# TuringLang/Bijectors.jl

Measured on NVIDIA H100. Metric: samples/sec: with_logabsdet_jacobian through 8-layer Planar flow, D=128, higher is better.
Workload: dtype f32

## Files before the change

bijectors.jl_b200/csrc/b2b_planar_const.cu:

```cuda
#include "b2b_planar_common.cuh"

namespace b2b {

template <int D>
struct PlanarHP {
  float v[2 * HP_MAX_L * D + 2 * HP_MAX_L];
};

template <int D>
struct ArgSrc {
  static constexpr bool kDerive = false;
  const PlanarHP<D>& H;
  int invmask;
  __device__ __forceinline__ bool inv(int l) const { return (invmask >> l) & 1; }
};

struct DevSrc {
  static constexpr bool kDerive = true;
  int invmask;
  __device__ __forceinline__ bool inv(int l) const { return (invmask >> l) & 1; }
};

template <int D, int DIR, bool MVN, class Src>
struct PlanarProg {
  using State = V1NoState;
  const Src src;
  const B2BChainParams& P;
  const int L;
  static constexpr bool DERIVE = Src::kDerive;
  static constexpr bool TAB = DERIVE && DIR != 0;
  __device__ __forceinline__ int npk() const { return 2 * L * D + 2 * L; }
  __device__ __forceinline__ int mvn_off() const { return (npk() + 3) & ~3; }
  __device__ __forceinline__ int tab_off() const { return mvn_off() + (MVN ? 2 * D + 4 : 0); }

  __device__ __forceinline__ void stage(float* params, int warp, int lane, int nw) const {
    if constexpr (DERIVE) {
      if (MVN && warp == nw - 1) stage_layer(P.layers[L], params + mvn_off(), D, D, lane);
      planar_derive_smem<D>(P, L, L, params, warp, lane, nw);
      if constexpr (TAB) {
        __syncthreads();
        for (int idx = warp * 32 + lane; idx < L * PT_N; idx += nw * 32) {
          const int l = idx / PT_N;
          if (DIR == 1 || src.inv(l)) planar_table_piece(params[2 * L * D + l], idx - l * PT_N, params + tab_off() + l * PT_FLOATS);
        }
      }
    } else {
      for (int i = warp * 32 + lane; i < npk(); i += nw * 32) params[i] = src.H.v[i];
    }
  }

  __device__ __forceinline__ void apply(float2 (&x)[1][D / 2], const ColCtx<D, 1>& ctx, const float* params,
                                        float (&lj)[1]) const {
    const float* cb = params + 2 * L * D;
    const float* tab = params + tab_off();
#pragma unroll 1
    for (int l = 0; l < L; ++l) {
      const float4* w4 = reinterpret_cast<const float4*>(params + l * D);
      const float4* u4 = reinterpret_cast<const float4*>(params + (L + l) * D);
      float2 acc[4];
#pragma unroll
      for (int i = 0; i < 4; ++i) acc[i] = make_float2(0.f, 0.f);
#pragma unroll
      for (int i = 0; i < D / 4; ++i) {
        const float4 w = w4[i];
        acc[(i & 1) * 2 + 0] = b2b_ffma2(make_float2(w.x, w.y), x[0][2 * i], acc[(i & 1) * 2 + 0]);
        acc[(i & 1) * 2 + 1] = b2b_ffma2(make_float2(w.z, w.w), x[0][2 * i + 1], acc[(i & 1) * 2 + 1]);
      }
      const float2 s = b2b_fadd2(b2b_fadd2(acc[0], acc[1]), b2b_fadd2(acc[2], acc[3]));
      const float wz = s.x + s.y;
      const float cc_ = cb[l], bb = cb[L + l];
      float t, s2;
      if (DIR == 0 || (DIR == 2 && !src.inv(l))) {
        tanh_sech2(wz + bb, t, s2);
        lj[0] += log1pf(cc_ * s2);
      } else {
        if constexpr (TAB) find_alpha_tab(wz, cc_, bb, tab + l * PT_FLOATS, t, s2);
        else find_alpha_ts(wz, cc_, bb, t, s2);
        lj[0] -= log1pf(cc_ * s2);
        t = -t;
      }
      const float2 t2 = make_float2(t, t);
#pragma unroll
      for (int i = 0; i < D / 4; ++i) {
        const float4 u = u4[i];
        x[0][2 * i] = b2b_ffma2(make_float2(u.x, u.y), t2, x[0][2 * i]);
        x[0][2 * i + 1] = b2b_ffma2(make_float2(u.z, u.w), t2, x[0][2 * i + 1]);
      }
    }
    if (MVN) mvnormal_apply<D, 1, 1>(x, ctx, params + mvn_off(), lj);
  }
};

template <int D, int NW, int DIR>
__global__ void __launch_bounds__(NW * 32, 1)
    planar_arg_kernel(const __grid_constant__ B2BChainParams P, const __grid_constant__ V1Extra E,
                      const __grid_constant__ CUtensorMap map_x, const __grid_constant__ CUtensorMap map_y,
                      const __grid_constant__ PlanarHP<D> H, const int L, const int invmask) {
  const PlanarProg<D, DIR, false, ArgSrc<D>> prog{{H, invmask}, P, L};
  v1_run<D, 1, 1, NW>(P, E, map_x, map_y, prog);
}

template <int D, int NW, int DIR, bool MVN>
__global__ void __launch_bounds__(NW * 32, 1)
    planar_dev_kernel(const __grid_constant__ B2BChainParams P, const __grid_constant__ V1Extra E,
                      const __grid_constant__ CUtensorMap map_x, const __grid_constant__ CUtensorMap map_y,
                      const int L, const int invmask) {
  const PlanarProg<D, DIR, MVN, DevSrc> prog{{invmask}, P, L};
  v1_run<D, 1, 1, NW>(P, E, map_x, map_y, prog);
}

template <int D, int NW, int DIR>
static int launch_arg(const B2BChainParams& q, const V1Geom& g, const CUtensorMap& mx, const CUtensorMap& my, int L,
                      const float* packed, int invmask, cudaStream_t stream) {
  static PlanarHP<D> H;
  static std::mutex mu;
  std::lock_guard<std::mutex> lock(mu);
  memcpy(H.v, packed, sizeof(float) * (size_t)(2 * L * D + 2 * L));
  auto kernel = planar_arg_kernel<D, NW, DIR>;
  cudaError_t e = cudaFuncSetAttribute(kernel, cudaFuncAttributeMaxDynamicSharedMemorySize, (int)g.smem);
  if (e != cudaSuccess) return (int)e;
  kernel<<<g.grid, NW * 32, g.smem, stream>>>(q, g.extra, mx, my, H, L, invmask);
  return (int)cudaGetLastError();
}

template <int D, int NW, int DIR, bool MVN = false>
static int launch_dev(const B2BChainParams& q, const V1Geom& g, const CUtensorMap& mx, const CUtensorMap& my, int L,
                      int invmask, cudaStream_t stream) {
  auto kernel = planar_dev_kernel<D, NW, DIR, MVN>;
  cudaError_t e = cudaFuncSetAttribute(kernel, cudaFuncAttributeMaxDynamicSharedMemorySize, (int)g.smem);
  if (e != cudaSuccess) return (int)e;
  kernel<<<g.grid, NW * 32, g.smem, stream>>>(q, g.extra, mx, my, L, invmask);
  return (int)cudaGetLastError();
}

template <int D, int NW>
static int dispatch(int L, const B2BChainParams& q, const V1Geom& g, const CUtensorMap& mx, const CUtensorMap& my,
                    const float* packed, int invmask, bool mvn, cudaStream_t stream) {
  const int all = (1 << L) - 1;
  const int dir = (invmask & all) == 0 ? 0 : ((invmask & all) == all ? 1 : 2);
  if (packed) {
    if (dir == 0) return launch_arg<D, NW, 0>(q, g, mx, my, L, packed, invmask, stream);
    if (dir == 1) return launch_arg<D, NW, 1>(q, g, mx, my, L, packed, invmask, stream);
    return launch_arg<D, NW, 2>(q, g, mx, my, L, packed, invmask, stream);
  }
  if (mvn) {
    if (dir == 1) return launch_dev<D, NW, 1, true>(q, g, mx, my, L, invmask, stream);
    return B2B_EUNSUPPORTED;
  }
  if (dir == 0) return launch_dev<D, NW, 0>(q, g, mx, my, L, invmask, stream);
  if (dir == 1) return launch_dev<D, NW, 1>(q, g, mx, my, L, invmask, stream);
  return launch_dev<D, NW, 2>(q, g, mx, my, L, invmask, stream);
}

static int launch_planar(const B2BChainParams& p, int L, const float* packed, int invmask, bool mvn,
                                  cudaStream_t stream) {
  B2BChainParams q = p;
  q.scratch_off = -1;
  if (!(q.D == 32 || q.D == 64 || q.D == 128) || L < 1 || L > HP_MAX_L) return B2B_EUNSUPPORTED;
  if (v1_check_io(q) != 0) return B2B_EUNSUPPORTED;
  V1Geom g;
  const size_t pf = (size_t)((2 * L * q.D + 2 * L + 3) & ~3) + (mvn ? 2 * q.D + 4 : 0) +
                    ((!packed && invmask != 0) ? (size_t)L * PT_FLOATS : 0);
  const int rc = v1_geometry(q.D, q.N, hp_warps(q.D), 32, pf, g);
  if (rc != 0) return rc;
  CUtensorMap mx, my;
  if (!make_maps(q, g.cols, &mx, &my, &g.extra.tma3d)) return B2B_EUNSUPPORTED;
  if (q.D == 128) return dispatch<128, 8>(L, q, g, mx, my, packed, invmask, mvn, stream);
  if (q.D == 64) return dispatch<64, 12>(L, q, g, mx, my, packed, invmask, mvn, stream);
  return dispatch<32, 16>(L, q, g, mx, my, packed, invmask, mvn, stream);
}

}

int b2b_planar_const_grid_size(const B2BChainParams& p) {
  using namespace b2b;
  if (!(p.D == 32 || p.D == 64 || p.D == 128)) return 0;
  V1Geom g;
  if (v1_geometry(p.D, p.N, hp_warps(p.D), 32, 0, g) != 0) return 0;
  return g.grid;
}

int b2b_launch_planar_hostparams(const B2BChainParams& p, int L, const float* packed, int invmask,
                                 cudaStream_t stream) {
  return b2b::launch_planar(p, L, packed, invmask, false, stream);
}

int b2b_planar_const_layers(const B2BChainParams& p) {
  using namespace b2b;
  if (!(p.D == 32 || p.D == 64 || p.D == 128) || p.L < 1) return 0;
  const bool mvn = p.layers[p.L - 1].kind == B2B_MVNORMAL_DIAG;
  const int n = p.L - (mvn ? 1 : 0);
  if (n < 1 || n > HP_MAX_L) return 0;
  for (int l = 0; l < n; ++l) {
    if (p.layers[l].kind != B2B_PLANAR) return 0;
    if (mvn && !p.layers[l].inverse) return 0;
  }
  if (v1_check_io(p) != 0) return 0;
  return n;
}

int b2b_launch_planar_chain_const(const B2BChainParams& p, cudaStream_t stream) {
  using namespace b2b;
  const int n = b2b_planar_const_layers(p);
  if (n == 0) return B2B_EUNSUPPORTED;
  int invmask = 0;
  for (int l = 0; l < n; ++l)
    if (p.layers[l].inverse) invmask |= 1 << l;
  return launch_planar(p, n, nullptr, invmask, p.L > n, stream);
}
```

bijectors.jl_b200/csrc/b2b_v1_pipeline.cuh:

```cuda
#pragma once
#include <cuda.h>
#include <cuda_runtime.h>

#include <cstdlib>
#include <mutex>

#include "b2b_device.cuh"

namespace b2b {

__device__ __forceinline__ uint32_t smem_u32(const void* p) {
  return static_cast<uint32_t>(__cvta_generic_to_shared(p));
}
__device__ __forceinline__ void mbar_init(uint32_t bar, uint32_t count) {
  asm volatile("mbarrier.init.shared::cta.b64 [%0], %1;" ::"r"(bar), "r"(count));
}
__device__ __forceinline__ void mbar_expect_tx(uint32_t bar, uint32_t bytes) {
  asm volatile("mbarrier.arrive.expect_tx.shared::cta.b64 _, [%0], %1;" ::"r"(bar), "r"(bytes) : "memory");
}
__device__ __forceinline__ void mbar_wait(uint32_t bar, uint32_t parity) {
  asm volatile(
      "{\n"
      ".reg .pred P1;\n"
      "B2B_WAIT:\n"
      "mbarrier.try_wait.parity.shared::cta.b64 P1, [%0], %1;\n"
      "@P1 bra B2B_DONE;\n"
      "bra B2B_WAIT;\n"
      "B2B_DONE:\n"
      "}\n" ::"r"(bar),
      "r"(parity)
      : "memory");
}
__device__ __forceinline__ void tma_load_2d(uint32_t dst, const CUtensorMap* map, int c0, int c1, uint32_t bar) {
  asm volatile(
      "cp.async.bulk.tensor.2d.shared::cluster.global.mbarrier::complete_tx::bytes [%0], [%1, {%2, %3}], [%4];" ::"r"(dst),
      "l"(reinterpret_cast<uint64_t>(map)), "r"(c0), "r"(c1), "r"(bar)
      : "memory");
}
__device__ __forceinline__ void tma_store_2d(const CUtensorMap* map, int c0, int c1, uint32_t src, uint64_t pol) {
  asm volatile("cp.async.bulk.tensor.2d.global.shared::cta.bulk_group.L2::cache_hint [%0, {%1, %2}], [%3], %4;" ::"l"(
                   reinterpret_cast<uint64_t>(map)),
               "r"(c0), "r"(c1), "r"(src), "l"(pol)
               : "memory");
}
__device__ __forceinline__ void tma_load_3d(uint32_t dst, const CUtensorMap* map, int c0, int c1, int c2, uint32_t bar) {
  asm volatile(
      "cp.async.bulk.tensor.3d.shared::cluster.global.mbarrier::complete_tx::bytes [%0], [%1, {%2, %3, %4}], [%5];" ::"r"(dst),
      "l"(reinterpret_cast<uint64_t>(map)), "r"(c0), "r"(c1), "r"(c2), "r"(bar)
      : "memory");
}
__device__ __forceinline__ void tma_store_3d(const CUtensorMap* map, int c0, int c1, int c2, uint32_t src, uint64_t pol) {
  asm volatile("cp.async.bulk.tensor.3d.global.shared::cta.bulk_group.L2::cache_hint [%0, {%1, %2, %3}], [%4], %5;" ::"l"(
                   reinterpret_cast<uint64_t>(map)),
               "r"(c0), "r"(c1), "r"(c2), "r"(src), "l"(pol)
               : "memory");
}
__device__ __forceinline__ uint64_t l2_evict_first() {
  uint64_t p;
  asm volatile("createpolicy.fractional.L2::evict_first.b64 %0, 1.0;" : "=l"(p));
  return p;
}
__device__ __forceinline__ void mbar_arrive(uint32_t bar) {
  asm volatile("mbarrier.arrive.shared::cta.b64 _, [%0];" ::"r"(bar) : "memory");
}
__device__ __forceinline__ void bulk_load_1d(uint32_t dst, const void* src, uint32_t bytes, uint32_t bar) {
  asm volatile("cp.async.bulk.shared::cluster.global.mbarrier::complete_tx::bytes [%0], [%1], %2, [%3];" ::"r"(dst),
               "l"(reinterpret_cast<uint64_t>(src)), "r"(bytes), "r"(bar)
               : "memory");
}
__device__ __forceinline__ void tma_commit() { asm volatile("cp.async.bulk.commit_group;" ::: "memory"); }
__device__ __forceinline__ void tma_wait_read0() { asm volatile("cp.async.bulk.wait_group.read 0;" ::: "memory"); }
__device__ __forceinline__ void tma_wait_all0() { asm volatile("cp.async.bulk.wait_group 0;" ::: "memory"); }
__device__ __forceinline__ void fence_proxy_async() { asm volatile("fence.proxy.async.shared::cta;" ::: "memory"); }
__device__ __forceinline__ void fence_mbar_init() { asm volatile("fence.mbarrier_init.release.cluster;" ::: "memory"); }
__device__ __forceinline__ void flag_store_release(int* p, int v) {
  asm volatile("st.release.cta.shared::cta.s32 [%0], %1;" ::"r"(smem_u32(p)), "r"(v) : "memory");
}
__device__ __forceinline__ int flag_load_acquire(const int* p) {
  int v;
  asm volatile("ld.acquire.cta.shared::cta.s32 %0, [%1];" : "=r"(v) : "r"(smem_u32(p)) : "memory");
  return v;
}

struct V1Extra {
  int n_in;
  int param_off;
  int bar_off;
  int nwarps;
  int tma3d;
  long long tiles;
};

template <int D, int TPC>
struct ColCtx {
  static constexpr int EPT = D / TPC;
  static constexpr int NQT = EPT / 32;
  int h, rot;
  __device__ __forceinline__ int prm(int ql, int r) const { return (h * NQT + ql) * 8 + (r ^ rot); }
  __device__ __forceinline__ int row(int ql, int r, int e) const { return prm(ql, r) * 4 + e; }
};

template <int TPC>
__device__ __forceinline__ float part_sum(float v) {
#pragma unroll
  for (int o = 1; o < TPC; o <<= 1) v += __shfl_xor_sync(0xffffffffu, v, o);
  return v;
}

#define B2B_FOR_SLOTS                        \
  _Pragma("unroll") for (int ql = 0; ql < C::NQT; ++ql) _Pragma("unroll") for (int r = 0; r < 8; ++r)
#define B2B_FOR_COLS _Pragma("unroll") for (int cc = 0; cc < CPT; ++cc)

template <int D, int TPC, int CPT>
__device__ __forceinline__ void radial_apply(float2 (&x)[CPT][D / TPC / 2], const ColCtx<D, TPC>& c, const float* sp,
                                             bool inverse, float (&lj)[CPT]) {
  using C = ColCtx<D, TPC>;
  const float4* z4 = reinterpret_cast<const float4*>(sp);
  const float alpha = sp[D], bhat = sp[D + 1], apb = sp[D + 2];
  const float2 m1 = make_float2(-1.f, -1.f);
  float2 acc[CPT][4];
  B2B_FOR_COLS {
#pragma unroll
    for (int i = 0; i < 4; ++i) acc[cc][i] = make_float2(0.f, 0.f);
  }
  B2B_FOR_SLOTS {
    const float4 z0 = z4[c.prm(ql, r)];
    const int i = (ql * 8 + r) * 2;
    B2B_FOR_COLS {
      const float2 d0 = b2b_ffma2(make_float2(z0.x, z0.y), m1, x[cc][i]);
      const float2 d1 = b2b_ffma2(make_float2(z0.z, z0.w), m1, x[cc][i + 1]);
      acc[cc][(r & 1) * 2 + 0] = b2b_ffma2(d0, d0, acc[cc][(r & 1) * 2 + 0]);
      acc[cc][(r & 1) * 2 + 1] = b2b_ffma2(d1, d1, acc[cc][(r & 1) * 2 + 1]);
    }
  }
  float2 g2[CPT];
  B2B_FOR_COLS {
    const float2 s = b2b_fadd2(b2b_fadd2(acc[cc][0], acc[cc][1]), b2b_fadd2(acc[cc][2], acc[cc][3]));
    const float nrm = sqrtf(part_sum<TPC>(s.x + s.y));
    float r_ = nrm;
    if (inverse) {
      const float a = apb - nrm;
      const float sq = sqrtf(fmaf(a, a, 4.0f * alpha * nrm));
      r_ = a > 0.f ? (2.0f * alpha * nrm) / (sq + a) : 0.5f * (sq - a);
    }
    const float hh = 1.0f / (alpha + r_);
    const float bh = bhat * hh;
    const float ljf = (float)(D - 1) * log1pf(bh) + log1pf(bh * alpha * hh);
    float g;
    if (!inverse) {
      g = bh;
      lj[cc] += ljf;
    } else {
      g = -bhat / (apb + r_);
      lj[cc] -= ljf;
    }
    g2[cc] = make_float2(g, g);
  }
  B2B_FOR_SLOTS {
    const float4 z0 = z4[c.prm(ql, r)];
    const int i = (ql * 8 + r) * 2;
    B2B_FOR_COLS {
      const float2 d0 = b2b_ffma2(make_float2(z0.x, z0.y), m1, x[cc][i]);
      const float2 d1 = b2b_ffma2(make_float2(z0.z, z0.w), m1, x[cc][i + 1]);
      x[cc][i] = b2b_ffma2(g2[cc], d0, x[cc][i]);
      x[cc][i + 1] = b2b_ffma2(g2[cc], d1, x[cc][i + 1]);
    }
  }
}

template <int D, int TPC, int CPT>
__device__ __forceinline__ void mvnormal_apply(const float2 (&x)[CPT][D / TPC / 2], const ColCtx<D, TPC>& c,
                                               const float* sp, float (&lj)[CPT]) {
  using C = ColCtx<D, TPC>;
  const float4* mu4 = reinterpret_cast<const float4*>(sp);
  const float4* is4 = reinterpret_cast<const float4*>(sp + D);
  const float2 m1 = make_float2(-1.f, -1.f);
  float2 acc[CPT][2];
  B2B_FOR_COLS acc[cc][0] = acc[cc][1] = make_float2(0.f, 0.f);
  B2B_FOR_SLOTS {
    const float4 mu = mu4[c.prm(ql, r)], is = is4[c.prm(ql, r)];
    const int i = (ql * 8 + r) * 2;
    B2B_FOR_COLS {
      const float2 z0 = b2b_fmul2(b2b_ffma2(make_float2(mu.x, mu.y), m1, x[cc][i]), make_float2(is.x, is.y));
      const float2 z1 = b2b_fmul2(b2b_ffma2(make_float2(mu.z, mu.w), m1, x[cc][i + 1]), make_float2(is.z, is.w));
      acc[cc][0] = b2b_ffma2(z0, z0, acc[cc][0]);
      acc[cc][1] = b2b_ffma2(z1, z1, acc[cc][1]);
    }
  }
  B2B_FOR_COLS {
    const float2 s = b2b_fadd2(acc[cc][0], acc[cc][1]);
    lj[cc] += sp[2 * D] - 0.5f * part_sum<TPC>(s.x + s.y);
  }
}

struct V1Gen {
  unsigned long long seed, offset;
  long long col0;
  const float* mu;
  const float* sigma;
};

__device__ __forceinline__ void philox4x32_10(uint32_t c0, uint32_t c1, uint32_t c2, uint32_t c3, uint32_t k0, uint32_t k1,
                                              uint32_t (&out)[4]) {
#pragma unroll
  for (int r = 0; r < 10; ++r) {
    const uint32_t hi0 = __umulhi(0xD2511F53u, c0), lo0 = 0xD2511F53u * c0;
    const uint32_t hi1 = __umulhi(0xCD9E8D57u, c2), lo1 = 0xCD9E8D57u * c2;
    c0 = hi1 ^ c1 ^ k0;
    c1 = lo1;
    c2 = hi0 ^ c3 ^ k1;
    c3 = lo0;
    k0 += 0x9E3779B9u;
    k1 += 0xBB67AE85u;
  }
  out[0] = c0;
  out[1] = c1;
  out[2] = c2;
  out[3] = c3;
}

__device__ __forceinline__ void box_muller(uint32_t a, uint32_t b, float& z0, float& z1) {
  const float u1 = fmaf(__uint2float_rn(a), 2.3283064365386963e-10f, 1.1641532182693481e-10f);
  const float u2 = fmaf(__uint2float_rn(b), 2.3283064365386963e-10f, 1.1641532182693481e-10f);
  const float r = sqrtf(-1.3862943611198906f * __log2f(u1));
  const float ang = 6.283185307179586f * u2 - 3.141592653589793f;
  z0 = -r * __cosf(ang);
  z1 = -r * __sinf(ang);
}

__device__ __forceinline__ float4 philox_normal4(const V1Gen& g, long long n, int k) {
  uint32_t o[4];
  philox4x32_10((uint32_t)n, (uint32_t)((unsigned long long)n >> 32), (uint32_t)k, (uint32_t)g.offset, (uint32_t)g.seed,
                (uint32_t)(g.seed >> 32), o);
  float4 z;
  box_muller(o[0], o[1], z.x, z.y);
  box_muller(o[2], o[3], z.z, z.w);
  return z;
}

struct V1NoState {};

template <int D, int TPC, int CPT, int NW, class Prog, int NIN = 1, bool GEN = false>
__device__ __forceinline__ void v1_run(const B2BChainParams& P, const V1Extra& E, const CUtensorMap& map_x,
                                       const CUtensorMap& map_y, const Prog& prog,
                                       const CUtensorMap* map_x2 = nullptr, const V1Gen* gen = nullptr) {
  using C = ColCtx<D, TPC>;
  constexpr int NQ = D / 32;
  constexpr int LPC = 32 / TPC;
  constexpr int COLS = LPC * CPT;
  constexpr int BOX_BYTES = COLS * 128;
  constexpr int TILE_BYTES = NQ * BOX_BYTES;
  constexpr int SLOT_BYTES = NIN * TILE_BYTES;
  extern __shared__ unsigned char smem_dyn[];
  unsigned char* smem_raw = smem_dyn + ((1024u - (smem_u32(smem_dyn) & 1023u)) & 1023u);
  unsigned char* in_base = smem_raw;
  unsigned char* out_base = smem_raw + (size_t)E.n_in * SLOT_BYTES;
  float* params = reinterpret_cast<float*>(smem_raw + E.param_off);
  uint64_t* bars = reinterpret_cast<uint64_t*>(smem_raw + E.bar_off);
  int* armed = reinterpret_cast<int*>(bars + 8);

  const int lane = threadIdx.x & 31, warp = __shfl_sync(0xffffffffu, (int)(threadIdx.x >> 5), 0);
  auto load_tile = [&](uint32_t dst, int col0, uint32_t bar) {
    if (E.tma3d) {
      tma_load_3d(dst, &map_x, 0, col0, 0, bar);
      if (NIN == 2) tma_load_3d(dst + TILE_BYTES, map_x2, 0, col0, 0, bar);
    } else {
#pragma unroll
      for (int q = 0; q < NQ; ++q) tma_load_2d(dst + q * BOX_BYTES, &map_x, q * 32, col0, bar);
      if (NIN == 2) {
#pragma unroll
        for (int q = 0; q < NQ; ++q) tma_load_2d(dst + TILE_BYTES + q * BOX_BYTES, map_x2, q * 32, col0, bar);
      }
    }
  };
  const long long my_tiles = (E.tiles - blockIdx.x + gridDim.x - 1) / gridDim.x;
  if (threadIdx.x == 0 && !GEN) {
    for (int i = 0; i < E.n_in; ++i) mbar_init(smem_u32(&bars[i]), 1);
    fence_mbar_init();
    for (int j = 0; j < E.n_in && j < my_tiles; ++j) {
      const uint32_t bar = smem_u32(&bars[j]);
      mbar_expect_tx(bar, SLOT_BYTES);
      const long long tile = blockIdx.x + (long long)j * gridDim.x;
      load_tile(smem_u32(in_base + (size_t)j * SLOT_BYTES), (int)(tile * COLS), bar);
      flag_store_release(&armed[j], j);
    }
  }
  prog.stage(params, warp, lane, NW);
  __syncthreads();

  C ctx;
  const int t = lane / TPC;
  ctx.h = lane % TPC;
  ctx.rot = ctx.h * (8 / TPC);
  unsigned char* my_out = out_base + (size_t)warp * TILE_BYTES;
  const int sw = (((t & 7) ^ ctx.rot) & 7) * 16;
  const int line = t * 128 + ctx.h * C::NQT * BOX_BYTES;
  double dsum = 0.0;
  bool store_pending = false;

  for (long long j = warp; j < my_tiles; j += NW) {
    const int buf = (int)(j % E.n_in);
    const uint32_t parity = (uint32_t)((j / E.n_in) & 1);
    const long long tile = blockIdx.x + j * gridDim.x;
    const long long col = tile * COLS + t;
    if constexpr (!GEN) {
      while (flag_load_acquire(&armed[buf]) != (int)j) __nanosleep(20);
      mbar_wait(smem_u32(&bars[buf]), parity);
    }

    float2 x[CPT][C::EPT / 2];
    auto load_fragment = [&](const unsigned char* src) {
      B2B_FOR_COLS {
        B2B_FOR_SLOTS {
          const float4 v =
              *reinterpret_cast<const float4*>(src + cc * (LPC * 128) + ql * BOX_BYTES + ((r * 16) ^ sw));
          x[cc][(ql * 8 + r) * 2] = make_float2(v.x, v.y);
          x[cc][(ql * 8 + r) * 2 + 1] = make_float2(v.z, v.w);
        }
      }
    };
    if constexpr (GEN) {
      B2B_FOR_COLS {
        const long long n = gen->col0 + col + cc * LPC;
        B2B_FOR_SLOTS {
          const int row0 = ctx.row(ql, r, 0);
          float4 z = philox_normal4(*gen, n, row0 >> 2);
          if (gen->sigma) {
            const float4 sg = __ldg(reinterpret_cast<const float4*>(gen->sigma + row0));
            z = make_float4(z.x * sg.x, z.y * sg.y, z.z * sg.z, z.w * sg.w);
          }
          if (gen->mu) {
            const float4 m = __ldg(reinterpret_cast<const float4*>(gen->mu + row0));
            z = make_float4(z.x + m.x, z.y + m.y, z.z + m.z, z.w + m.w);
          }
          x[cc][(ql * 8 + r) * 2] = make_float2(z.x, z.y);
          x[cc][(ql * 8 + r) * 2 + 1] = make_float2(z.z, z.w);
        }
      }
    } else {
      load_fragment(in_base + (size_t)buf * SLOT_BYTES + line);
    }
    typename Prog::State st;
    if constexpr (NIN == 2) {
      prog.phase1(x, ctx, params, st);
      load_fragment(in_base + (size_t)buf * SLOT_BYTES + TILE_BYTES + line);
    }
    if constexpr (!GEN) fence_proxy_async();
    __syncwarp();
    if (!GEN && lane == 0 && j + E.n_in < my_tiles) {
      const uint32_t bar = smem_u32(&bars[buf]);
      mbar_expect_tx(bar, SLOT_BYTES);
      const long long nt = blockIdx.x + (j + E.n_in) * gridDim.x;
      load_tile(smem_u32(in_base + (size_t)buf * SLOT_BYTES), (int)(nt * COLS), bar);
      flag_store_release(&armed[buf], (int)(j + E.n_in));
    }

    float lj[CPT];
    B2B_FOR_COLS {
      const long long cl = col + cc * LPC;
      lj[cc] = (P.accumulate && P.logjac && cl < P.N) ? P.logjac[cl] : 0.0f;
    }
    if constexpr (NIN == 2) prog.apply(x, ctx, params, lj, st, col);
    else prog.apply(x, ctx, params, lj);

    if (P.y) {
      if (store_pending) {
        if (lane == 0) tma_wait_read0();
        __syncwarp();
      }
      unsigned char* dst = my_out + line;
      B2B_FOR_COLS {
        B2B_FOR_SLOTS {
          const float2 a = x[cc][(ql * 8 + r) * 2], b = x[cc][(ql * 8 + r) * 2 + 1];
          *reinterpret_cast<float4*>(dst + cc * (LPC * 128) + ql * BOX_BYTES + ((r * 16) ^ sw)) =
              make_float4(a.x, a.y, b.x, b.y);
        }
      }
      fence_proxy_async();
      __syncwarp();
      if (lane == 0) {
        const uint64_t pol = l2_evict_first();
        if (E.tma3d) {
          tma_store_3d(&map_y, 0, (int)(tile * COLS), 0, smem_u32(my_out), pol);
        } else {
#pragma unroll
          for (int q = 0; q < NQ; ++q)
            tma_store_2d(&map_y, q * 32, (int)(tile * COLS), smem_u32(my_out + q * BOX_BYTES), pol);
        }
        tma_commit();
      }
      store_pending = true;
    }
    if (ctx.h == 0) {
      B2B_FOR_COLS {
        const long long cl = col + cc * LPC;
        if (cl < P.N) {
          if (P.logjac && !(P.accumulate & 2)) P.logjac[cl] = lj[cc];
          dsum += (double)lj[cc];
        }
      }
    }
  }
  if (lane == 0 && store_pending) tma_wait_all0();

  if (P.partials) {
    __shared__ double red[32];
#pragma unroll
    for (int o = 16; o > 0; o >>= 1) dsum += __shfl_xor_sync(0xffffffffu, dsum, o);
    if (lane == 0) red[warp] = dsum;
    __syncthreads();
    if (threadIdx.x == 0) {
      double tt = 0.0;
      for (int w = 0; w < NW; ++w) tt += red[w];
      P.partials[blockIdx.x] = tt;
    }
  }
}

typedef CUresult (*encode_tiled_fn)(CUtensorMap*, CUtensorMapDataType, cuuint32_t, void*, const cuuint64_t*,
                                    const cuuint64_t*, const cuuint32_t*, const cuuint32_t*, CUtensorMapInterleave,
                                    CUtensorMapSwizzle, CUtensorMapL2promotion, CUtensorMapFloatOOBfill);

static inline encode_tiled_fn get_encode() {
  static encode_tiled_fn fn = nullptr;
  static std::once_flag once;
  std::call_once(once, [] {
    void* p = nullptr;
    cudaDriverEntryPointQueryResult q;
    if (cudaGetDriverEntryPoint("cuTensorMapEncodeTiled", &p, cudaEnableDefault, &q) == cudaSuccess &&
        q == cudaDriverEntryPointSuccess)
      fn = reinterpret_cast<encode_tiled_fn>(p);
  });
  return fn;
}

static inline bool make_map(CUtensorMap* m, const float* base, int D, long long N, long long ld, int cols, bool three_d) {
  encode_tiled_fn enc = get_encode();
  if (!enc) return false;
  const cuuint32_t estr[3] = {1, 1, 1};
  if (three_d) {
    const cuuint64_t dims[3] = {32, (cuuint64_t)N, (cuuint64_t)(D / 32)};
    const cuuint64_t strides[2] = {(cuuint64_t)ld * sizeof(float), 128};
    const cuuint32_t box[3] = {32, (cuuint32_t)cols, (cuuint32_t)(D / 32)};
    return enc(m, CU_TENSOR_MAP_DATA_TYPE_FLOAT32, 3, const_cast<float*>(base), dims, strides, box, estr,
               CU_TENSOR_MAP_INTERLEAVE_NONE, CU_TENSOR_MAP_SWIZZLE_128B, CU_TENSOR_MAP_L2_PROMOTION_L2_128B,
               CU_TENSOR_MAP_FLOAT_OOB_FILL_NONE) == CUDA_SUCCESS;
  }
  const cuuint64_t dims[2] = {(cuuint64_t)D, (cuuint64_t)N};
  const cuuint64_t strides[1] = {(cuuint64_t)ld * sizeof(float)};
  const cuuint32_t box[2] = {32, (cuuint32_t)cols};
  return enc(m, CU_TENSOR_MAP_DATA_TYPE_FLOAT32, 2, const_cast<float*>(base), dims, strides, box, estr,
             CU_TENSOR_MAP_INTERLEAVE_NONE, CU_TENSOR_MAP_SWIZZLE_128B, CU_TENSOR_MAP_L2_PROMOTION_L2_128B,
             CU_TENSOR_MAP_FLOAT_OOB_FILL_NONE) == CUDA_SUCCESS;
}

static inline bool make_maps(const B2BChainParams& q, int cols, CUtensorMap* mx, CUtensorMap* my, int* tma3d) {
  for (int three_d = 1; three_d >= 0; --three_d) {
    if (three_d && q.D == 32) continue;
    bool ok = make_map(mx, q.x, q.D, q.N, q.ldx, cols, three_d != 0);
    if (ok && q.y) ok = make_map(my, q.y, q.D, q.N, q.ldy, cols, three_d != 0);
    if (ok) {
      if (!q.y) *my = *mx;
      *tma3d = three_d;
      return true;
    }
  }
  return false;
}

struct V1Geom {
  int nw, grid, cols;
  size_t smem;
  V1Extra extra;
};

static inline int v1_check_io(const B2BChainParams& p) {
  if (p.N >= (1ll << 31) - 64) return B2B_EUNSUPPORTED;
  if ((p.ldx % 4) || (reinterpret_cast<uintptr_t>(p.x) & 15)) return B2B_EUNSUPPORTED;
  if (p.y && ((p.ldy % 4) || (reinterpret_cast<uintptr_t>(p.y) & 15))) return B2B_EUNSUPPORTED;
  return 0;
}

static inline int v1_geometry(int D, long long N, int nw, int cols, size_t param_floats, V1Geom& g,
                              int in_tiles = 1) {
  const int tile_bytes = D * 4 * cols;
  const size_t param_bytes = param_floats * sizeof(float);
  const size_t budget = 225 * 1024;
  const size_t fixed = (size_t)nw * tile_bytes + ((param_bytes + 15) & ~(size_t)15) + 16 * sizeof(uint64_t) + 1024;
  const size_t slot_bytes = (size_t)in_tiles * tile_bytes;
  if (fixed + 2 * slot_bytes > budget) return B2B_EUNSUPPORTED;
  int n_in = (int)((budget - fixed) / slot_bytes);
  if (n_in > 8) n_in = 8;
  g.nw = nw;
  g.cols = cols;
  g.extra.n_in = n_in;
  g.extra.nwarps = nw;
  g.extra.tma3d = 0;
  g.extra.param_off = n_in * (int)slot_bytes + nw * tile_bytes;
  g.extra.bar_off = g.extra.param_off + (int)((param_bytes + 15) & ~(size_t)15);
  g.extra.tiles = (N + cols - 1) / cols;
  g.smem = (size_t)g.extra.bar_off + 16 * sizeof(uint64_t) + 1024;
  const int sms = b2b_sm_count();
  long long grid = sms;
  const long long want = (g.extra.tiles + nw - 1) / nw;
  if (grid > want) grid = want;
  if (grid < 1) grid = 1;
  g.grid = (int)grid;
  return 0;
}

}
```

Baseline: 2.657 billion.

## Split tile schedule into persistent main CTAs plus extra tail CTAs

Changes the persistent-grid tile schedule so that one CTA per SM handles about 7/8 of the tiles in strided order. The remaining tiles go to a set of additional CTAs, capped at a maximum grid size, each taking a small chunk. This is meant to reduce tail imbalance at the end of the persistent loop. It adds more CTA launches and prologue/param-staging cost, and is only enabled for host-param or forward-only planar configurations.

```diff
diff --git a/bijectors.jl_b200/csrc/b2b_planar_const.cu b/bijectors.jl_b200/csrc/b2b_planar_const.cu
--- a/bijectors.jl_b200/csrc/b2b_planar_const.cu
+++ b/bijectors.jl_b200/csrc/b2b_planar_const.cu
@@ -152,6 +152,8 @@
   return launch_dev<D, NW, 2>(q, g, mx, my, L, invmask, stream);
 }
 
+static bool planar_tail(bool host_params, int invmask) { return host_params || invmask == 0; }
+
 static int launch_planar(const B2BChainParams& p, int L, const float* packed, int invmask, bool mvn,
                                   cudaStream_t stream) {
   B2BChainParams q = p;
@@ -161,7 +163,7 @@
   V1Geom g;
   const size_t pf = (size_t)((2 * L * q.D + 2 * L + 3) & ~3) + (mvn ? 2 * q.D + 4 : 0) +
                     ((!packed && invmask != 0) ? (size_t)L * PT_FLOATS : 0);
-  const int rc = v1_geometry(q.D, q.N, hp_warps(q.D), 32, pf, g);
+  const int rc = v1_geometry(q.D, q.N, hp_warps(q.D), 32, pf, g, 1, planar_tail(packed != nullptr, invmask));
   if (rc != 0) return rc;
   CUtensorMap mx, my;
   if (!make_maps(q, g.cols, &mx, &my, &g.extra.tma3d)) return B2B_EUNSUPPORTED;
@@ -175,8 +177,12 @@
 int b2b_planar_const_grid_size(const B2BChainParams& p) {
   using namespace b2b;
   if (!(p.D == 32 || p.D == 64 || p.D == 128)) return 0;
+  int invmask = 0;
+  if (b2b_planar_const_layers(p) > 0)
+    for (int l = 0; l < p.L; ++l)
+      if (p.layers[l].kind == B2B_PLANAR && p.layers[l].inverse) invmask |= 1 << l;
   V1Geom g;
-  if (v1_geometry(p.D, p.N, hp_warps(p.D), 32, 0, g) != 0) return 0;
+  if (v1_geometry(p.D, p.N, hp_warps(p.D), 32, 0, g, 1, planar_tail(false, invmask)) != 0) return 0;
   return g.grid;
 }
 
diff --git a/bijectors.jl_b200/csrc/b2b_v1_pipeline.cuh b/bijectors.jl_b200/csrc/b2b_v1_pipeline.cuh
--- a/bijectors.jl_b200/csrc/b2b_v1_pipeline.cuh
+++ b/bijectors.jl_b200/csrc/b2b_v1_pipeline.cuh
@@ -88,6 +88,8 @@
   int bar_off;
   int nwarps;
   int tma3d;
+  int main_ctas;
+  long long main_tiles;
   long long tiles;
 };
 
@@ -273,14 +275,20 @@
       }
     }
   };
-  const long long my_tiles = (E.tiles - blockIdx.x + gridDim.x - 1) / gridDim.x;
+  long long t0 = blockIdx.x, tstride = E.main_ctas, tend = E.main_tiles;
+  if ((int)blockIdx.x >= E.main_ctas) {
+    t0 = E.main_tiles + (blockIdx.x - E.main_ctas);
+    tstride = gridDim.x - E.main_ctas;
+    tend = E.tiles;
+  }
+  const long long my_tiles = tend > t0 ? (tend - t0 + tstride - 1) / tstride : 0;
   if (threadIdx.x == 0 && !GEN) {
     for (int i = 0; i < E.n_in; ++i) mbar_init(smem_u32(&bars[i]), 1);
     fence_mbar_init();
     for (int j = 0; j < E.n_in && j < my_tiles; ++j) {
       const uint32_t bar = smem_u32(&bars[j]);
       mbar_expect_tx(bar, SLOT_BYTES);
-      const long long tile = blockIdx.x + (long long)j * gridDim.x;
+      const long long tile = t0 + (long long)j * tstride;
       load_tile(smem_u32(in_base + (size_t)j * SLOT_BYTES), (int)(tile * COLS), bar);
       flag_store_release(&armed[j], j);
     }
@@ -301,7 +309,7 @@
   for (long long j = warp; j < my_tiles; j += NW) {
     const int buf = (int)(j % E.n_in);
     const uint32_t parity = (uint32_t)((j / E.n_in) & 1);
-    const long long tile = blockIdx.x + j * gridDim.x;
+    const long long tile = t0 + j * tstride;
     const long long col = tile * COLS + t;
     if constexpr (!GEN) {
       while (flag_load_acquire(&armed[buf]) != (int)j) __nanosleep(20);
@@ -350,7 +358,7 @@
     if (!GEN && lane == 0 && j + E.n_in < my_tiles) {
       const uint32_t bar = smem_u32(&bars[buf]);
       mbar_expect_tx(bar, SLOT_BYTES);
-      const long long nt = blockIdx.x + (j + E.n_in) * gridDim.x;
+      const long long nt = t0 + (j + E.n_in) * tstride;
       load_tile(smem_u32(in_base + (size_t)buf * SLOT_BYTES), (int)(nt * COLS), bar);
       flag_store_release(&armed[buf], (int)(j + E.n_in));
     }
@@ -468,6 +476,7 @@
   return false;
 }
 
+constexpr int V1_MAX_GRID = 4096;
 struct V1Geom {
   int nw, grid, cols;
   size_t smem;
@@ -482,7 +491,7 @@
 }
 
 static inline int v1_geometry(int D, long long N, int nw, int cols, size_t param_floats, V1Geom& g,
-                              int in_tiles = 1) {
+                              int in_tiles = 1, bool tail = true) {
   const int tile_bytes = D * 4 * cols;
   const size_t param_bytes = param_floats * sizeof(float);
   const size_t budget = 225 * 1024;
@@ -506,6 +515,16 @@
   if (grid > want) grid = want;
   if (grid < 1) grid = 1;
   g.grid = (int)grid;
+  g.extra.main_ctas = (int)grid;
+  g.extra.main_tiles = g.extra.tiles;
+  const long long per = g.extra.tiles * 7 / (8 * grid);
+  if (tail && grid == sms && per >= 8 * nw) {
+    const long long rest = g.extra.tiles - per * grid;
+    long long chunk = nw;
+    if ((rest + chunk - 1) / chunk > V1_MAX_GRID - grid) chunk = (rest + V1_MAX_GRID - grid - 1) / (V1_MAX_GRID - grid);
+    g.extra.main_tiles = per * grid;
+    g.grid = (int)(grid + (rest + chunk - 1) / chunk);
+  }
   return 0;
 }
 
```

New measurement: 2.705 billion (median of 6 runs). 1.02x the previous value.
